# ChalmersPhotonicsLab/QAMpy

Hardware: AMD Instinct MI355X
Metric: equalised MSym/s (2-pol, 2 SPS) (higher is better)
Workload: dtype f32

## Files before the change

### qampy_amd/csrc/api.hip

```cpp
#include "common.h"
#include <stdlib.h>
#include <atomic>
#include <mutex>
#include <vector>
#include <unordered_map>
#include <string.h>

namespace qh {

thread_local hipStream_t g_stream = nullptr;
static thread_local hipStream_t g_streams[4] = {nullptr, nullptr, nullptr, nullptr};
int g_device = -1;
static thread_local std::string g_err;
static std::mutex g_mu;

void set_error(const std::string &s) { g_err = s; }

int hip_fail(hipError_t e, const char *what, const char *file, int line)
{
    g_err = std::string(hipGetErrorString(e)) + " in " + what + " (" + file + ":" + std::to_string(line) + ")";
    (void)hipGetLastError();
    return QH_ERR_HIP;
}

// ... 63 lines not shown
        QH_HIP(hipStreamCreateWithPriority(&g_streams[i], hipStreamNonBlocking, i == 2 ? prio_least : prio_greatest));
    }
    g_stream = g_streams[0];
    g_device = device;
    return QH_OK;
}

hipStream_t side_stream() { return g_stream == g_streams[0] ? g_streams[1] : g_streams[0]; }
hipStream_t helper_stream() { return g_streams[3]; }

int ensure_init()
{
    if (g_stream) return QH_OK;
    return init_device(g_device >= 0 ? g_device : 0);
}

thread_local void *g_scratch[SCRATCH_SLOTS] = {nullptr};
thread_local size_t g_scratch_n[SCRATCH_SLOTS] = {0};
thread_local unsigned g_scratch_epoch = 0;
static std::atomic<int> g_form[FORM_COUNT];
struct FormName { const char *key, *env; };
static const FormName FORM_NAMES[FORM_COUNT] = {
    {"trainer", "QAMPY_HIP_TRAINER"}, {"pit_form", "QAMPY_HIP_PIT_FORM"}, {"seg_lanes", "QAMPY_HIP_SEG_LANES"}, {"pit_probe", "QAMPY_HIP_PIT_PROBE"},
    {"bps", "QAMPY_HIP_BPS"}, {"pit_tail", "QAMPY_HIP_PIT_TAIL"}};
static int form_parse(int k, const char *v, int *out)
{
    if (!v || !v[0]) { *out = 0; return 0; }
    switch (k) {
    case FORM_TRAINER: *out = v[0] == 'd' ? 1 : (v[0] == 'l' ? 2 : (v[0] == 'i' ? 3 : (v[0] == 'a' || v[0] == '0' ? 0 : -1))); break;
    case FORM_PIT: *out = v[0] == 's' ? 1 : (v[0] == 'b' ? 2 : (v[0] == 'a' || v[0] == '0' ? 0 : -1)); break;
    case FORM_SEG_LANES: { const int n = atoi(v); *out = (n == 8 || n == 16 || n == 0) ? n : -1; break; }
    case FORM_BPS: *out = v[0] == 't' ? 1 : (v[0] == 'l' ? 2 : (v[0] == 'a' || v[0] == '0' ? 0 : -1)); break;
    case FORM_PIT_TAIL: *out = v[0] == 's' ? 1 : (v[0] == 'a' || v[0] == '0' ? 0 : -1); break;
    default: *out = atoi(v) != 0 ? 1 : 0; break;
    }
    return *out < 0 ? -1 : 0;
}
static const int g_form_env_read = [] {
    for (int k = 0; k < FORM_COUNT; k++) {
        int v = 0;
        if (form_parse(k, getenv(FORM_NAMES[k].env), &v) == 0) g_form[k].store(v);
    }
    return 0;
}();
int form(FormKey k) { return g_form[k].load(std::memory_order_relaxed); }
const char *trainer_force()
{
    switch (form(FORM_TRAINER)) {
    case 1: return "direct";
    case 2: return "lookahead";
    case 3: return "iterative";
    default: return "";
    }
}
static constexpr int POOL_CLASSES = 48, POOL_KEEP = 8;
static constexpr size_t POOL_BYTES = (size_t)24 << 30;
// ... 370 lines not shown
```

### qampy_amd/csrc/common.h

```cpp
#pragma once
#include <hip/hip_runtime.h>
#include <stdint.h>
#include <string>
#include "../../include/qampy_hip.h"

namespace qh {

extern thread_local hipStream_t g_stream;
extern int g_device;
void set_error(const std::string &s);
int hip_fail(hipError_t e, const char *what, const char *file, int line);

#define QH_HIP(call)                                                        \
    do {                                                                    \
        hipError_t _e = (call);                                             \
        if (_e != hipSuccess) return qh::hip_fail(_e, #call, __FILE__, __LINE__); \
    } while (0)

#define QH_REQUIRE(cond, msg)                                   \
    do {                                                        \
        if (!(cond)) { qh::set_error(msg); return QH_ERR_ARG; } \
    } while (0)

#define QH_WAVE_FIRST() __builtin_amdgcn_s_setprio(3)

int ensure_init();
hipStream_t side_stream();
hipStream_t helper_stream();
enum FormKey { FORM_TRAINER = 0, FORM_PIT, FORM_SEG_LANES, FORM_PIT_PROBE, FORM_BPS, FORM_PIT_TAIL, FORM_COUNT };
int form(FormKey k);
const char *trainer_force();
double gram_budget_gb();
int pit_timing_mode();
int default_tier();
double default_tier_tol();
constexpr int SCRATCH_SLOTS = 24;
constexpr int SCRATCH_TWOSTAGE = 16;
constexpr int SCRATCH_FOE = 17;
constexpr int SCRATCH_IMPAIR = 18;
constexpr int SCRATCH_PMD = 19;
constexpr int SCRATCH_TXRESP = 20;
constexpr int SCRATCH_SOS = 21;
constexpr int SCRATCH_CPR = 22;
constexpr int SCRATCH_FFT = 23;
int scratch(int slot, size_t bytes, void **p);
unsigned scratch_epoch();

int bps_twostage_recover_f32(const void *E, int nm, int64_t L, const void *angles, int A, int B, const void *symbols, int M, int N, int32_t *idx1,
                             int32_t *idx2, void *ph, void *Eout);
int bps_twostage_recover_f64(const void *E, int nm, int64_t L, const void *angles, int A, int B, const void *symbols, int M, int N, int32_t *idx1,
                             int32_t *idx2, void *ph, void *Eout);

// ... 114 lines not shown
```

### qampy_amd/csrc/train_pit.h

```cpp
#pragma once
#include <atomic>
#include <chrono>
#include <vector>
#include "train_impl.h"
#include "train_seg.h"

namespace qh {

typedef qh_pit_report PitCtrl;

constexpr double PIT_CONTRACT = 0.2;
constexpr int PIT_PROBE = 128;
constexpr int PIT_SEEDWIN = 512;
constexpr int PIT_MAXSEG = 65536;

__host__ __device__ inline int pit_symmetry(int method)
{
    switch (method) {
    case QH_M_CMA: case QH_M_SGNCMA: case QH_M_RDE: return 0;
    case QH_M_CMA2: return 2;
    default: return 4;
    }
}

// ... 27 lines not shown
    if (lane == 63) buf[wave] = x;
    __syncthreads();
    T pre = ident;
    for (int w = 0; w < wave; w++) pre = op(pre, buf[w]);
    T ex = shfl_up_any(x, 1);
    if (lane == 0) ex = ident;
    const T r = op(pre, ex);
    __syncthreads();
    return r;
}

template <typename T> __device__ __forceinline__ void block_prefix_sum(T *a, int n, T *tot)
{
    const int len = (n + 255) / 256;
    const int i0 = threadIdx.x * len, i1 = i0 + len < n ? i0 + len : n;
    T s = 0;
    for (int i = i0; i < i1; i++) s += a[i];
    T run = block_scan_excl<T>(s, [](T x, T y) { return x + y; }, (T)0, tot);
    for (int i = i0; i < i1; i++) { run += a[i]; a[i] = run; }
    __syncthreads();
}

template <typename R>
__global__ void __launch_bounds__(256) pit_setup_kernel(const Cx<R> *E, int nmodes, int64_t L, int64_t npow, int ntot, const R *mu, double gear,
                                                        double bound, double tol, PitSeg sg, PitCtrl *c, R *mu_acq)
{
    QH_WAVE_FIRST();
    __shared__ double red[256];
    double acc = 0;
    for (int k = 0; k < nmodes; k++)
        for (int64_t i = threadIdx.x; i < npow; i += 256) {
            const Cx<R> v = E[(size_t)k * L + i];
            acc += (double)v.re * v.re + (double)v.im * v.im;
        }
    red[threadIdx.x] = acc;
    __syncthreads();
    for (int s = 128; s > 0; s >>= 1) {
        if (threadIdx.x < s) red[threadIdx.x] += red[threadIdx.x + s];
        __syncthreads();
    }
    if (threadIdx.x == 0) {
        const double p = red[0] / ((double)nmodes * (double)npow);
        const double m = (double)*mu;
        double ma = gear * m;
        const double cap = bound / ((double)ntot * (p > 1e-30 ? p : 1e-30));
        if (ma > cap) ma = cap;
        if (!(ma > m)) ma = m;
        c->segments = sg.S; c->seg_len = sg.len; c->mu = m; c->mu_acq = ma; c->power = p; c->tol = tol;
        for (int q = 0; q < QH_PIT_MAXPASS; q++) { c->result_change[q] = -1; c->deviation[q] = -1; c->deviation_rms[q] = -1; c->deviation_taps[q] = -1; c->deviation_taps_worst[q] = -1; } c->passes = 0; c->converged = 0; c->acq_chunks = 0; c->acq_steps = 0; c->acq_done = 0; c->done = 0; c->diverged = 0; c->corr_on = 0; c->gain = 0; c->out_power = 0;
        for (int i = 0; i < QH_PIT_MAXPASS; i++) c->defect[i] = -1;
        for (int i = 0; i < QH_PIT_MAXCHUNK; i++) c->acq_err[i] = -1;
        *mu_acq = (R)ma;
    }
}

template <typename R>
__global__ void __launch_bounds__(256) pit_acq_monitor_kernel(const Cx<R> *err, int64_t err_pitch, int64_t step0, int64_t n, int nsel,
                                                              const int64_t *modes_dev, double plateau, PitCtrl *c, R *mu_acq, const R *mu, double floor_gear)
{
    QH_WAVE_FIRST();
    if (threadIdx.x == 0 && floor_gear >= 0) {
        const R lo = (R)((double)*mu * floor_gear), h = *mu_acq * (R)0.5;
        *mu_acq = h > lo ? h : (*mu_acq > lo ? lo : *mu_acq);
    }
    if (c->acq_done) return;
    __shared__ double red[256];
    double acc = 0;
    for (int j = 0; j < nsel; j++) {
        const Cx<R> *row = err + (size_t)modes_dev[j] * err_pitch + step0;
        for (int64_t i = threadIdx.x; i < n; i += 256) {
            const Cx<R> v = row[i];
            acc += (double)v.re * v.re + (double)v.im * v.im;
        }
    }
    red[threadIdx.x] = acc;
    __syncthreads();
    for (int s = 128; s > 0; s >>= 1) {
// ... 2 lines not shown
    }
    if (threadIdx.x == 0) {
        const double v = red[0] / ((double)n * nsel);
        const int k = c->acq_chunks;
        if (k < QH_PIT_MAXCHUNK) c->acq_err[k] = v;
        c->acq_chunks = k + 1;
        c->acq_steps = step0 + n;
        if (!(v == v) || v > 1e30) { c->diverged = 1; c->acq_done = 1; return; }
        if (k >= 1) {
            const double prev = c->acq_err[k - 1 < QH_PIT_MAXCHUNK ? k - 1 : QH_PIT_MAXCHUNK - 1];
            if (v > 100 * c->acq_err[0]) { c->diverged = 1; c->acq_done = 1; return; }
            if (v > plateau * prev) c->acq_done = 1;
        }
    }
}

template <typename R> __global__ void pit_acq_finish_kernel(Cx<R> *wx, const Cx<R> *w_start, int n, PitCtrl *c)
{
    QH_WAVE_FIRST();
    const int i = blockIdx.x * blockDim.x + threadIdx.x;
    if (c->diverged && i < n) wx[i] = w_start[i];
}

inline size_t pit_phase_pitch(int ntaps, int os, int nwin) { return (size_t)nwin + (size_t)(ntaps + os - 1) / os + 1; }
template <typename R>
__global__ void __launch_bounds__(256) pit_phase_kernel(const Cx<R> *E, int nmodes, int64_t L, int os, const Cx<R> *wx, int ntaps, PitSeg sg,
                                                        const int64_t *modes_dev, int nwin, double *z)
{
    QH_WAVE_FIRST();
    extern __shared__ __attribute__((aligned(16))) char pit_smem[];
    Cx<R> *w = reinterpret_cast<Cx<R> *>(pit_smem);
    const int ntot = nmodes * ntaps;
    const int pitch = nwin + (ntaps + os - 1) / os + 1;
    Cx<R> *xs = w + ntot;
    __shared__ double rr[256], ri[256];
    const int s = blockIdx.x, j = blockIdx.y;
    const int mode = (int)modes_dev[j];
    for (int f = threadIdx.x; f < ntot; f += 256) w[f] = wx[(size_t)mode * ntot + f];
    const int64_t st = sg.start(s);
    int64_t n = sg.steps(s);
    if (n > nwin) n = nwin;
    const int ns = n > 0 ? (int)(n - 1) * os + ntaps : 0;
    for (int k = 0; k < nmodes; k++) {
        const Cx<R> *x = E + (size_t)k * L + st * os;
        for (int g = threadIdx.x; g < ns; g += 256) xs[((size_t)k * os + g % os) * pitch + g / os] = x[g];
    }
    __syncthreads();
    double zr = 0, zi = 0;
    for (int i = threadIdx.x; i < n; i += 256) {
        R yr = 0, yi = 0;
        for (int k = 0; k < nmodes; k++) {
            const Cx<R> *wk = w + k * ntaps;
            for (int r = 0; r < os; r++) {
                const Cx<R> *xp = xs + ((size_t)k * os + r) * pitch + i;
                int u = 0;
                for (int t = r; t < ntaps; t += os, u++) {
                    const Cx<R> a = xp[u], b = wk[t];
                    yr = fma_(a.re, b.re, fma_(-a.im, b.im, yr));
                    yi = fma_(a.re, b.im, fma_(a.im, b.re, yi));
                }
            }
        }
        const double y2r = (double)yr * yr - (double)yi * yi, y2i = 2.0 * yr * yi;
        zr += y2r * y2r - y2i * y2i;
        zi += 2.0 * y2r * y2i;
    }
    rr[threadIdx.x] = zr; ri[threadIdx.x] = zi;
    __syncthreads();
    for (int q = 128; q > 0; q >>= 1) {
        if (threadIdx.x < q) { rr[threadIdx.x] += rr[threadIdx.x + q]; ri[threadIdx.x] += ri[threadIdx.x + q]; }
        __syncthreads();
    }
    if (threadIdx.x == 0) { z[2 * ((size_t)s * gridDim.y + j)] = rr[0]; z[2 * ((size_t)s * gridDim.y + j) + 1] = ri[0]; }
}

static __global__ void __launch_bounds__(256) pit_unwrap_kernel(const double *z, int S, int nsel, double *rot, double *phi, int *jump)
{
    QH_WAVE_FIRST();
    __shared__ int ptot[512];
    const double q = 1.5707963267948966;
    phi += (size_t)blockIdx.x * S; jump += (size_t)blockIdx.x * S;
    for (int j = blockIdx.x; j <= (int)blockIdx.x; j++) {
        for (int s = threadIdx.x; s < S; s += 256) {
            const double zr = z[2 * ((size_t)s * nsel + j)], zi = z[2 * ((size_t)s * nsel + j) + 1];
            phi[s] = (zr == 0 && zi == 0) ? 0.0 : (double)atan2f((float)-zi, (float)-zr) / 4;
        }
        __syncthreads();
        for (int s = threadIdx.x; s < S; s += 256) jump[s] = s == 0 ? 0 : (int)rint((phi[s - 1] - phi[s]) / q);
        __syncthreads();
        block_prefix_sum<int>(jump, S, ptot);
        for (int s = threadIdx.x; s < S; s += 256) {
            const double p = phi[s] + q * (jump[s] & 3);
            float sn, cs;
            sincosf((float)p, &sn, &cs);
            rot[2 * ((size_t)s * nsel + j)] = cs;
            rot[2 * ((size_t)s * nsel + j) + 1] = -sn;
        }
        __syncthreads();
    }
}

template <typename R>
__global__ void __launch_bounds__(256) pit_seed_kernel(const Cx<R> *wx, int nmodes, int ntot, const int64_t *modes_dev, int nsel, const double *rot, Cx<R> *X,
                                                       const Cx<R> *w0, Cx<R> *Y, PitCtrl *c)
{
    QH_WAVE_FIRST();
    const int s = blockIdx.x;
    const int n = nmodes * ntot;
    if (s == 0 && c) {
        if (threadIdx.x == 0) { c->done = 0; c->converged = 0; c->passes = 0; }
        for (int q = threadIdx.x; q < QH_PIT_MAXPASS; q += 256) {
            c->result_change[q] = -1; c->deviation[q] = -1; c->deviation_rms[q] = -1; c->deviation_taps[q] = -1; c->deviation_taps_worst[q] = -1; c->defect[q] = -1;
        }
    }
    const bool exact0 = s == 0 && w0 != nullptr;
    for (int e = threadIdx.x; e < n; e += 256) {
        const int row = e / ntot;
        Cx<R> v = exact0 ? w0[e] : wx[e];
        if (rot && !exact0) {
            for (int j = 0; j < nsel; j++)
                if ((int)modes_dev[j] == row) {
                    const double c = rot[2 * ((size_t)s * nsel + j)], d = rot[2 * ((size_t)s * nsel + j) + 1];
                    const double vr = (double)v.re * c - (double)v.im * d, vi = (double)v.re * d + (double)v.im * c;
                    v = Cx<R>{(R)vr, (R)vi};
                    break;
                }
        }
        X[(size_t)s * n + e] = v;
        Y[(size_t)s * n + e] = v;
    }
}

template <typename R>
__global__ void __launch_bounds__(PIT_PROBE) pit_defect_kernel(const Cx<R> *E, int nmodes, int64_t L, int os, int ntaps, PitSeg sg, int64_t TrSyms,
                                                                const int64_t *modes_dev, const Cx<R> *X, const Cx<R> *Y, int sym, const PitCtrl *c, double *dfc, double *pw, double *gph,
                                                                const Cx<R> *wx_prev)
{
    QH_WAVE_FIRST();
    if (c->done) return;
    extern __shared__ __attribute__((aligned(16))) char pit_smem[];
    Cx<R> *wa = reinterpret_cast<Cx<R> *>(pit_smem);
    const int ntot = nmodes * ntaps;
    Cx<R> *wb = wa + ntot;
    const int pitch = PIT_PROBE + (ntaps + os - 1) / os + 1;
    Cx<R> *xs = wb + ntot;
    __shared__ double red[4][PIT_PROBE];
    const int b = blockIdx.x + 1, j = blockIdx.y;
    const int mode = (int)modes_dev[j];
    const size_t wset = (size_t)nmodes * ntot;
    const bool result_probe = b == sg.S;
    for (int f = threadIdx.x; f < ntot; f += PIT_PROBE) {
        wa[f] = result_probe ? wx_prev[(size_t)mode * ntot + f] : X[(size_t)b * wset + (size_t)mode * ntot + f];
        wb[f] = Y[(size_t)(b - 1) * wset + (size_t)mode * ntot + f];
// ... 1723 lines not shown

struct PitPrepLayout { size_t ctrl, mu_acq, modes, wx, w0, err, gram, total; int64_t err_pitch; };
template <typename R> inline PitPrepLayout pit_prep_layout(int nmodes, int ntaps, int64_t acq_steps)
{
    PitPrepLayout l;
    auto up = [](size_t x) { return (x + 255) / 256 * 256; };
    const size_t wset = (size_t)nmodes * nmodes * ntaps * sizeof(Cx<R>);
    l.err_pitch = (acq_steps + LA_B + 63) / 64 * 64;
    l.ctrl = 0; l.mu_acq = up(sizeof(PitCtrl)); l.modes = l.mu_acq + 64; l.wx = up(l.modes + 128); l.w0 = up(l.wx + wset);
    l.err = up(l.w0 + wset); l.gram = up(l.err + (size_t)nmodes * l.err_pitch * sizeof(Cx<R>));
    l.total = up(l.gram + gram_bytes<R>(l.err_pitch));
    return l;
}
template <typename R> __global__ void __launch_bounds__(256) pit_adopt_kernel(Cx<R> *wx, const Cx<R> *wx_prep, int n, const PitCtrl *p, PitCtrl *c, R *mu_acq, const R *mu_acq_prep)
{
    QH_WAVE_FIRST();
    const int i = blockIdx.x * blockDim.x + threadIdx.x;
    if (!p->diverged && i < n) wx[i] = wx_prep[i];
    if (i == 0) {
        c->acq_chunks = p->acq_chunks; c->acq_steps = p->acq_steps; c->acq_done = 1; c->diverged = p->diverged; c->mu_acq = p->mu_acq;
        for (int q = 0; q < QH_PIT_MAXCHUNK; q++) c->acq_err[q] = p->acq_err[q];
        *mu_acq = *mu_acq_prep;
    }
}
template <typename R>
int pit_prepare(const void *E, int nmodes, int64_t L, int64_t TrSyms, int os, const R *mu_dev, const void *wx0, int ntaps, const int64_t *modes, int nsel,
                const void *symbols, int64_t nsy, int method, const qh_pit_opts *opts, void *prep, size_t prep_bytes)
{
    int rc = ensure_init();
    if (rc) return rc;
    if ((rc = train_args_ok("pit prepare", method, nmodes, ntaps, os, TrSyms, 1, nsel, nsy, modes))) return rc;
    QH_REQUIRE(opts && prep, "pit prepare: options and a preparation buffer are needed");
    QH_REQUIRE(TrSyms >= 1, "pit prepare: bad sizes");
    QH_REQUIRE((TrSyms - 1) * os + ntaps <= L, "pit prepare: field shorter than TrSyms*os + ntaps");
    const qh_pit_opts &o = *opts;
    QH_REQUIRE(o.acquire != 0 && o.adaptive == 0 && o.segments > 1 && o.mu_hint > 0 && o.acq_chunk > 0 && o.head_steps == 0 && !o.exchange,
               "pit prepare: not preparable (a cold fixed-step sweep with segments, mu_hint and acq_chunk given)");
    const int ntot = nmodes * ntaps;
    const PitPlan pl = pit_plan(o, TrSyms, 0, o.segments, false, o.acq_chunk);
    const PitSeg &sg = pl.sg;
    QH_REQUIRE(sg.S >= 2, "pit prepare: not preparable (nothing to parallelise)");
    const char *not_prep = "pit prepare: not preparable (throughput-form passes, block-form acquisition, blind error function)";
    QH_REQUIRE(!(method == QH_M_SBD || method == QH_M_MDDMA || method == QH_M_DD || method == QH_M_SBD_DATA), not_prep);
    TrainerForm f;
    if ((rc = trainer_form<R>(f, FORM_PASSES, method, 0, nmodes, ntaps, os, sg.len, (int64_t)sg.S * nsel, symbols, nsy, modes, nsel))) return rc;
    QH_REQUIRE(f.seg && f.block && la_shape_ok(nmodes, ntaps, os), not_prep);
// ... 87 lines not shown
        QH_REQUIRE(!o.exchange, "train_equaliser: a capture split over processes takes no exact head");
        head = (int64_t)o.head_steps / LA_B * LA_B;
        if (head > TrSyms) head = TrSyms / LA_B * LA_B;
        o.acquire = 0;
    }
    int64_t seg_want = 2048;
    if (adaptive && !(method == QH_M_SBD || method == QH_M_MDDMA || method == QH_M_DD)) {
        const int64_t t = ((TrSyms - head) / 512 + LA_B - 1) / LA_B * LA_B;
        if (t > seg_want) seg_want = t;
    }
    if (S == 0 && adaptive) S = (int)((TrSyms - head) / seg_want < PIT_MAXSEG ? (TrSyms - head) / seg_want : PIT_MAXSEG);
    if (S == 0) {
        R mu_h = (R)o.mu_hint;
        if (!(o.mu_hint > 0)) {
            QH_HIP(hipMemcpyAsync(&mu_h, mu_dev, sizeof(R), hipMemcpyDeviceToHost, g_stream));
            QH_HIP(hipStreamSynchronize(g_stream));
        }
        S = pit_auto_segments(TrSyms, (double)mu_h, nsel, o.acquire);
    }
    PitPlan pl = pit_plan(o, TrSyms, head, S, adaptive, o.acquire ? o.acq_chunk : 0);
    const PitSeg &sg = pl.sg;
    if (zero_err) QH_HIP(hipMemsetAsync(err, 0, (size_t)nmodes * TrSyms * Niter * sizeof(Cx<R>), g_stream));
    const int64_t npow = L < 4096 ? L : 4096;
    hipLaunchKernelGGL((pit_setup_kernel<R>), dim3(1), dim3(256), 0, g_stream, (const Cx<R> *)E, nmodes, L, npow, ntot, (const R *)mu_dev, pl.gear, pl.bound, tol, sg, ctrl, mu_acq);
    QH_HIP(hipGetLastError());
    if (TrSyms == 0 || Niter == 0) return QH_OK;
    if (sg.S < 2) {
        const double zero = 0;
        QH_HIP(hipMemcpyAsync(&ctrl->defect[0], &zero, sizeof(double), hipMemcpyHostToDevice, g_stream));
        return exact_form(ctrl, adaptive ? 1 : 0, 0, gram, 1);
    }

    TrainerForm f;
    if ((rc = trainer_form<R>(f, FORM_PASSES, method, adaptive, nmodes, ntaps, os, sg.len, (int64_t)sg.S * nsel, symbols, nsy, modes, nsel))) return rc;
    if (adaptive && !f.seg) return exact_form(ctrl, 1, 0, nullptr, 0);
    const bool decision = method == QH_M_SBD || method == QH_M_MDDMA || method == QH_M_DD;
    const bool seg_form = f.seg, use_bi = f.use_bi, block_form = f.block, pair_tab = f.pair_tab;
    const bool split = o.exchange != nullptr;
    const int own_first = split ? o.seg_first : 0, own_count = split ? o.seg_count : sg.S;
    const bool xchg_async = split && o.exchange_on_stream != 0;
    if (split) {
        QH_REQUIRE(seg_form, "train_equaliser: a capture split over processes needs the throughput form of the passes (>= 512 chains, supported tap layout)");
        QH_REQUIRE(own_first >= 0 && own_count >= 0 && own_first + own_count <= sg.S, "train_equaliser: owned segments outside the segment grid");
        QH_REQUIRE(Niter == 1, "train_equaliser: a capture split over processes is trained in one sweep");
    }

    const size_t wset = (size_t)nmodes * ntot;
// ... 10 lines not shown
    float *devmax = (float *)(uw_jump + (size_t)sg.S * nsel);
    const int ndev = (int)((nsj + 63) / 64);
    unsigned *ticket = (unsigned *)(devmax + 4 * (size_t)ndev);
    PitInit init{};
    init.z[0] = ticket; init.zn[0] = sizeof(unsigned);
    R *ad_rS = nullptr, *ad_rE = nullptr;
    Cx<R> *ad_eS = nullptr, *ad_eE = nullptr, *ad_errh = nullptr;
    float *ad_M = nullptr, *ad_chg = nullptr, *ad_rP = nullptr, *ad_dP = nullptr;
    if (!adaptive && head > 0) {
        void *ab = nullptr;
        if ((rc = scratch(13, (size_t)nmodes * head * sizeof(Cx<R>) + 64, &ab))) return rc;
        ad_errh = (Cx<R> *)ab;
    }
    if (adaptive) {
        void *ab = nullptr;
        const size_t nS = ((size_t)sg.S + 15) / 16 * 16;
        if ((rc = scratch(13, nS * (2 * sizeof(R) + 2 * sizeof(Cx<R>) + 3 * sizeof(float)) + 64 + (size_t)nmodes * head * sizeof(Cx<R>), &ab))) return rc;
        ad_eS = (Cx<R> *)ab; ad_eE = ad_eS + nS; ad_errh = ad_eE + nS;
        ad_rS = (R *)(ad_errh + (size_t)nmodes * head); ad_rE = ad_rS + nS;
        ad_M = (float *)(ad_rE + nS); ad_rP = ad_M + nS; ad_dP = ad_rP + nS; ad_chg = ad_dP + nS;
    }
    init.modes_dev = modes_dev; init.nsel = nsel;
    for (int j = 0; j < 16; j++) init.modes[j] = j < nsel ? modes[j] : 0;
    const bool prepared = o.prepared != nullptr && o.acquire && !adaptive && head == 0 && Niter >= 1;
    const bool need_mu = adaptive || !(o.mu_hint > 0), need_acq = o.acquire && !(o.acq_chunk > 0) && !prepared;
    R mu_acq_h = 0;
    if (need_acq) QH_HIP(hipMemcpyAsync(&mu_acq_h, mu_acq, sizeof(R), hipMemcpyDeviceToHost, g_stream));
    R mu_host = need_mu ? (R)1 : (R)o.mu_hint;
    if (need_mu) QH_HIP(hipMemcpyAsync(&mu_host, mu_dev, sizeof(R), hipMemcpyDeviceToHost, g_stream));
    if (need_mu || need_acq) QH_HIP(hipStreamSynchronize(g_stream));
    if (!adaptive && !(mu_host != 0))
        return exact_form(ctrl, 0, 0, gram, 0);
    if (o.acquire && !(o.acq_chunk > 0)) pl.acquisition(o, TrSyms, pit_acq_chunk(mu_acq_h));

    const int64_t amax = pl.amax;
    void *G = const_cast<void *>(gram);
    if (prepared) QH_REQUIRE(seg_form && o.acq_chunk > 0, "train_equaliser: a prepared acquisition belongs to throughput-form passes with acq_chunk given (qh_pit_prepare_*_dev said so)");
    if (block_form && !G && (!seg_form || amax > 0) && !prepared) {
        const int64_t n = seg_form ? pl.ngram : TrSyms;
        rc = pair_tab ? gram_build<R>(E, nmodes, L, os, ntaps, n, &G) : gram_cur_build<R>(E, nmodes, L, os, ntaps, n, &G);
        if (rc) return rc;
    }
    const int64_t g_per_step = pair_tab ? LA_B : GRAM_TRI / 2 / LA_B;

    const int ncol = sg.S * nsel;
    const double *lam = nullptr;
    const Zf *Vb = nullptr;
    Zf *Dz[2] = {nullptr, nullptr};
// ... 40 lines not shown
        QH_HIP(hipFuncSetAttribute((const void *)pit_cgemm_kernel<R, true>, hipFuncAttributeMaxDynamicSharedMemorySize, 160 * 1024 - 256));
        QH_HIP(hipFuncSetAttribute((const void *)pit_cgemm_kernel<R, false>, hipFuncAttributeMaxDynamicSharedMemorySize, 160 * 1024 - 256));
        QH_HIP(hipFuncSetAttribute((const void *)pit_basis_mfma_kernel<R, 0>, hipFuncAttributeMaxDynamicSharedMemorySize, 128 * 1024));
        QH_HIP(hipFuncSetAttribute((const void *)pit_basis_mfma_kernel<R, 1>, hipFuncAttributeMaxDynamicSharedMemorySize, 128 * 1024));
        QH_HIP(hipFuncSetAttribute((const void *)pit_tail_kernel<R>, hipFuncAttributeMaxDynamicSharedMemorySize, 128 * 1024));
        gemm_attr.store(true, std::memory_order_release);
    }

    LaArgs<R> la = la_args<R>(E, L, nmodes, ntaps, os, modes, nsel, method, symbols, nsy, mu_dev, err, TrSyms * Niter);
    la.G = (const GramPair<R> *)G; la.gpair = pair_tab ? 1 : 0; la.wx_cs = (int64_t)wset;
    la.dd_general = f.dd_general;
    f.alphabet(la);
    const TrainArgs<R> ta = train_args<R>(E, L, nmodes, ntaps, os, TrSyms, Niter, modes, nsel, method, symbols, nsy, mu_dev, err);

    PitTiming &tm = pit_timing();
    tm.npass = 0; tm.acq_ms = 0;
    bool acq_timed = false;
    PitEvents &ev = pit_events();
    QH_REQUIRE(ev.ok, "train_equaliser: no pinned memory for the pass flags");
    const bool redo_ok = o.exact_redo_off == 0;
    bool fell_back = false;
    if (redo_ok && !adaptive) { init.cd[0] = w_call; init.cs[0] = wx; init.cn[0] = (unsigned)wbytes; }
    if (o.acquire && Niter > 0) { init.cd[1] = w_start; init.cs[1] = wx; init.cn[1] = (unsigned)wbytes; }
    hipLaunchKernelGGL(pit_init_kernel, dim3(32), dim3(256), 0, g_stream, init);
    QH_HIP(hipGetLastError());
    for (int it = 0; it < Niter; it++) {
        if (it == 0 && prepared) {
            const PitPrepLayout lay = pit_prep_layout<R>(nmodes, ntaps, amax);
            const char *pb = (const char *)o.prepared;
            hipLaunchKernelGGL((pit_adopt_kernel<R>), dim3((unsigned)((wset + 255) / 256)), dim3(256), 0, g_stream, (Cx<R> *)wx, (const Cx<R> *)(pb + lay.wx), (int)wset,
                               (const PitCtrl *)(pb + lay.ctrl), ctrl, mu_acq, (const R *)(pb + lay.mu_acq));
            QH_HIP(hipGetLastError());
        } else if (it == 0 && o.acquire) {
            if (pl.nchunks > 0) { QH_HIP(hipEventRecord(ev.t0[PIT_NEV - 1], g_stream)); acq_timed = true; }
            if ((rc = pit_acq_enqueue<R>(pl, block_form ? &la : nullptr, use_bi, &ta, (Cx<R> *)wx, (Cx<R> *)err, TrSyms * Niter, ctrl, mu_acq, mu_dev,
                                         modes_dev, nsel))) return rc;
            if (pl.nchunks > 0) QH_HIP(hipEventRecord(ev.t1[PIT_NEV - 1], g_stream));
            hipLaunchKernelGGL((pit_acq_finish_kernel<R>), dim3((unsigned)((wset + 255) / 256)), dim3(256), 0, g_stream, (Cx<R> *)wx, (const Cx<R> *)w_start, (int)wset, ctrl);
            QH_HIP(hipGetLastError());
        }
        if (adaptive) {
            QH_HIP(hipMemcpyAsync(w_start, wx, wbytes, hipMemcpyDeviceToDevice, g_stream));
            QH_HIP(hipMemcpyAsync(ad_chg + 1, mu_dev, sizeof(R), hipMemcpyDeviceToDevice, g_stream));
            if ((rc = train_dev<R>(E, nmodes, L, head, 1, os, mu_dev, wx, ntaps, modes, 1, 1, symbols, nsy, method, ad_errh, 0, nullptr))) return rc;
            QH_HIP(hipMemcpyAsync((Cx<R> *)err + (size_t)modes[0] * TrSyms, ad_errh + (size_t)modes[0] * head, (size_t)head * sizeof(Cx<R>), hipMemcpyDeviceToDevice, g_stream));
            hipLaunchKernelGGL((pit_adapt_init_kernel<R>), dim3((sg.S + 255) / 256), dim3(256), 0, g_stream, (const R *)mu_dev, (const Cx<R> *)(ad_errh + (size_t)modes[0] * head + head - 1),
                               sg.S, ad_rS, ad_eS);
            QH_HIP(hipGetLastError());
        }
        if (!adaptive && head > 0) {
            if ((rc = train_dev<R>(E, nmodes, L, head, 1, os, mu_dev, wx, ntaps, modes, nsel, 0, symbols, nsy, method, ad_errh, 0, nullptr))) return rc;
            for (int j = 0; j < nsel; j++)
                QH_HIP(hipMemcpyAsync((Cx<R> *)err + (size_t)modes[j] * TrSyms * Niter + (size_t)it * TrSyms, ad_errh + (size_t)modes[j] * head, (size_t)head * sizeof(Cx<R>),
                                      hipMemcpyDeviceToDevice, g_stream));
        }
        const double *rot_use = nullptr;
        if (seed_phase) {
            int nwin = PIT_SEEDWIN;
            auto phase_lds = [&](int nw) { return ((size_t)ntot + (size_t)nmodes * os * pit_phase_pitch(ntaps, os, nw)) * sizeof(Cx<R>); };
            while (nwin > 32 && phase_lds(nwin) > 60 * 1024) nwin /= 2;
            QH_REQUIRE(phase_lds(nwin) <= 60 * 1024, "train_equaliser: phase seeding does not fit the LDS for this filter shape (pass phase_seed = 0)");
            hipLaunchKernelGGL((pit_phase_kernel<R>), dim3(sg.S, nsel), dim3(256), phase_lds(nwin), g_stream, (const Cx<R> *)E, nmodes, L, os,
                               (const Cx<R> *)wx, ntaps, sg, (const int64_t *)modes_dev, nwin, z);
            hipLaunchKernelGGL(pit_unwrap_kernel, dim3(nsel), dim3(256), 0, g_stream, (const double *)z, sg.S, nsel, rot, uw_phi, uw_jump);
            rot_use = rot;
        }
        const Cx<R> *w_exact = o.start == 1 ? nullptr : ((it == 0 && o.acquire) ? (const Cx<R> *)w_start : (const Cx<R> *)wx);
        hipLaunchKernelGGL((pit_seed_kernel<R>), dim3(sg.S), dim3(256), 0, g_stream, (const Cx<R> *)wx, nmodes, ntot, (const int64_t *)modes_dev, nsel, rot_use, X, w_exact, Y, ctrl);
        if (ssb) {
            ma.sg = sg; ma.rot = rot_use;
            static thread_local hipEvent_t ev_seed = nullptr, ev_model = nullptr;
            if (!ev_seed) { QH_HIP(hipEventCreateWithFlags(&ev_seed, hipEventDisableTiming)); QH_HIP(hipEventCreateWithFlags(&ev_model, hipEventDisableTiming)); }
            hipStream_t ss = helper_stream();
            QH_HIP(hipEventRecord(ev_seed, g_stream));
            QH_HIP(hipStreamWaitEvent(ss, ev_seed, 0));
            hipLaunchKernelGGL((pit_model_kernel<R, 0>), dim3(PIT_MODB), dim3(256), 0, ss, ma);
            hipLaunchKernelGGL((pit_model_kernel<R, 1>), dim3(PIT_MODB), dim3(256), 0, ss, ma);
            QH_HIP(hipEventRecord(ev_model, ss));
            model_event = ev_model;
        }
        QH_HIP(hipGetLastError());
        const int timing_mode = pit_timing_mode();
        auto decide_args = [&](int p, const float *dm, const float2 *ye, float2 *yprev, int ne, int ncol_e, int corr_wanted) {
            PitDecideArgs<R> d;
            d.dfc = dfc; d.pw = pw; d.nb = (int)((sg.S - 1) * nsel); d.Ylast = (const Cx<R> *)(Y + (size_t)(sg.S - 1) * wset); d.n = (int)wset; d.wx = (Cx<R> *)wx; d.c = ctrl;
            d.host_view = &ev.hview[2 * p]; d.nrow = nsel; d.devmax = dm; d.ndev = ndev; d.safety = safety; d.Ye = ye; d.Yprev = yprev; d.ne = ne; d.ncol_e = ncol_e;
            d.theta = theta; d.modes_dev = (const int64_t *)modes_dev; d.ntot_w = ntot; d.S = (int)sg.S; d.sym = sym; d.corr_wanted = corr_wanted;
            d.extra = adaptive ? (const float *)ad_chg : nullptr;
            d.Dfin = (ye && !adaptive) ? (const float2 *)Dz[1] : nullptr; d.Vfin = (const float2 *)Vb; d.lam_fin = lam;
            d.stall_from = o.correction == 0 ? QH_PIT_MAXPASS : (adaptive ? 5 : 2);
            return d;
        };
        auto timed = [&](int p) { return timing_mode == 2 || (timing_mode == 1 && p == 1); };
        int back_done_for = 0;
        auto enqueue_pass = [&](int p) -> int {
            ((volatile float *)ev.hview)[2 * p] = -1.f;
            PitFuse<R> fz;
            fz.X = X; fz.Y = Y; fz.theta = theta; fz.modes_dev = (const int64_t *)modes_dev; fz.nmodes = nmodes; fz.nsel = nsel;
            fz.damp = (adaptive && p > 1) ? ad_damp : 1.f;
            fz.x_only = tail_fused ? 1 : 0;
            if (p > 0 && tail_fused && back_done_for == p) {
// ... 24 lines not shown
                for (int j = 0; j < 16; j++) sa.modes[j] = j < nsel ? modes[j] : 0;
                sa.skip = &ctrl->done;
                sa.q_first = own_first * nsel; sa.q_count = split ? own_count * nsel : 0;
                pit_last_launch().form = 1;
                if (!split || own_count > 0) { int r = launch_seg<R>(sa, method, adaptive); if (r) return r; }
                if (adaptive) hipLaunchKernelGGL((pit_adapt_scan_kernel<R>), dim3(1), dim3(1024), 0, g_stream, ad_rS, (const R *)ad_rE, ad_eS, (const Cx<R> *)ad_eE, sg.S, ad_chg, (const PitCtrl *)ctrl, ad_relax, ad_rP, ad_dP, ad_newton);
            } else if (block_form) {
                LaArgs<R> ls = la;
                ls.TrSyms = sg.len; ls.nch = sg.S; ls.wx = Y; ls.err_off = (int64_t)it * TrSyms; ls.seg = 1; ls.seg_extra = sg.extra; ls.seg_tail = sg.tail;
                ls.skip = &ctrl->done;
                pit_last_launch() = PitLaunch{use_bi ? 2 : 3, 0, 0, 0, 0, 0};
                if (sg.begin > 0) {
                    ls.E = (const Cx<R> *)E + sg.begin * os; ls.L = L - sg.begin * os; ls.err_off += sg.begin;
                    ls.G = (const GramPair<R> *)G + sg.begin * g_per_step;
                }
                { int r = use_bi ? launch_bi<R>(ls) : launch_la<R>(ls); if (r) return r; }
            } else {
                TrainArgs<R> ts = ta;
                ts.wx = Y; ts.nseg = sg.S; ts.seg_begin = sg.begin; ts.seg_len = sg.len; ts.seg_extra = sg.extra; ts.seg_tail = sg.tail; ts.seg_iter = it; ts.skip = &ctrl->done;
                pit_last_launch() = PitLaunch{4, 0, 0, 0, 0, 0};
                { int r = launch_any<R>(ts); if (r) return r; }
            }
            if (timed(p)) QH_HIP(hipEventRecord(ev.t1[p], g_stream));
            if (split) {
                if (own_first > 0) QH_HIP(hipMemsetAsync(Y, 0, (size_t)own_first * wbytes, g_stream));
                if (own_first + own_count < sg.S)
                    QH_HIP(hipMemsetAsync(Y + (size_t)(own_first + own_count) * wset, 0, (size_t)(sg.S - own_first - own_count) * wbytes, g_stream));
                if (!xchg_async) QH_HIP(hipStreamSynchronize(g_stream));
                if (o.exchange(o.exchange_user, Y, (size_t)sg.S * wbytes) != 0) { set_error("train_equaliser: the exchange callback failed"); return QH_ERR_ARG; }
            }
            const int nbnd = (int)((sg.S - 1) * nsel);
            if (eig) {
                if (o.basis && pit_basis_sync().pending) {
                    QH_HIP(hipStreamWaitEvent(g_stream, pit_basis_sync().out, 0));
                    pit_basis_sync().pending = false;
                }
                auto forward2 = [&](const Cx<R> *src, Zf *dst, const Cx<R> *src2, Zf *dst2) {
                    PitFuse<R> f2 = fz;
                    f2.T2 = src2; f2.Out2 = reinterpret_cast<float2 *>(dst2);
                    hipLaunchKernelGGL((pit_basis_mfma_kernel<R, 0>), dim3(2 * ((ncol + PIT_MC - 1) / PIT_MC)), dim3(pit_mfma_threads(ntot)), pit_mfma_lds(ntot), g_stream, Vb, src, (const Zf *)nullptr, dst, ntot, ncol, (const PitCtrl *)ctrl, f2);
                };
                if (p == 0 && model_event) QH_HIP(hipStreamWaitEvent(g_stream, model_event, 0));
                forward2((const Cx<R> *)X, Xe, (const Cx<R> *)Y, Ye);
                hipLaunchKernelGGL(pit_bound_kernel, dim3((nbnd + nsel + 3) / 4), dim3(256), 0, g_stream, (const Zf *)Xe, (const Zf *)Ye, (const Zf *)Yprev, lam, ntot, sg.S, nsel, sym,
                                   (const PitCtrl *)ctrl, dfc, pw, gph, ualpha);
                hipLaunchKernelGGL((pit_gauge_kernel<R>), dim3(ssb ? 2 : 1), dim3(PIT_GT_THREADS), 0, g_stream, (const double *)gph, sg.S, nsel, ctrl, theta, (const double *)pw,
// ... 194 lines not shown
```

Before: 1237.

## Merge PIT prologue kernels and add windowed phase-seed kernel

```diff
diff --git a/qampy_amd/csrc/api.hip b/qampy_amd/csrc/api.hip
--- a/qampy_amd/csrc/api.hip
+++ b/qampy_amd/csrc/api.hip
@@ -109,7 +109,7 @@
 struct FormName { const char *key, *env; };
 static const FormName FORM_NAMES[FORM_COUNT] = {
     {"trainer", "QAMPY_HIP_TRAINER"}, {"pit_form", "QAMPY_HIP_PIT_FORM"}, {"seg_lanes", "QAMPY_HIP_SEG_LANES"}, {"pit_probe", "QAMPY_HIP_PIT_PROBE"},
-    {"bps", "QAMPY_HIP_BPS"}, {"pit_tail", "QAMPY_HIP_PIT_TAIL"}};
+    {"bps", "QAMPY_HIP_BPS"}, {"pit_tail", "QAMPY_HIP_PIT_TAIL"}, {"pit_prologue", "QAMPY_HIP_PIT_PROLOGUE"}};
 static int form_parse(int k, const char *v, int *out)
 {
     if (!v || !v[0]) { *out = 0; return 0; }
@@ -118,7 +118,7 @@
     case FORM_PIT: *out = v[0] == 's' ? 1 : (v[0] == 'b' ? 2 : (v[0] == 'a' || v[0] == '0' ? 0 : -1)); break;
     case FORM_SEG_LANES: { const int n = atoi(v); *out = (n == 8 || n == 16 || n == 0) ? n : -1; break; }
     case FORM_BPS: *out = v[0] == 't' ? 1 : (v[0] == 'l' ? 2 : (v[0] == 'a' || v[0] == '0' ? 0 : -1)); break;
-    case FORM_PIT_TAIL: *out = v[0] == 's' ? 1 : (v[0] == 'a' || v[0] == '0' ? 0 : -1); break;
+    case FORM_PIT_TAIL: case FORM_PIT_PROLOGUE: *out = v[0] == 's' ? 1 : (v[0] == 'a' || v[0] == '0' ? 0 : -1); break;
     default: *out = atoi(v) != 0 ? 1 : 0; break;
     }
     return *out < 0 ? -1 : 0;
diff --git a/qampy_amd/csrc/common.h b/qampy_amd/csrc/common.h
--- a/qampy_amd/csrc/common.h
+++ b/qampy_amd/csrc/common.h
@@ -27,7 +27,7 @@
 int ensure_init();
 hipStream_t side_stream();
 hipStream_t helper_stream();
-enum FormKey { FORM_TRAINER = 0, FORM_PIT, FORM_SEG_LANES, FORM_PIT_PROBE, FORM_BPS, FORM_PIT_TAIL, FORM_COUNT };
+enum FormKey { FORM_TRAINER = 0, FORM_PIT, FORM_SEG_LANES, FORM_PIT_PROBE, FORM_BPS, FORM_PIT_TAIL, FORM_PIT_PROLOGUE, FORM_COUNT };
 int form(FormKey k);
 const char *trainer_force();
 double gram_budget_gb();
diff --git a/qampy_amd/csrc/train_pit.h b/qampy_amd/csrc/train_pit.h
--- a/qampy_amd/csrc/train_pit.h
+++ b/qampy_amd/csrc/train_pit.h
@@ -73,10 +73,9 @@
 }
 
 template <typename R>
-__global__ void __launch_bounds__(256) pit_setup_kernel(const Cx<R> *E, int nmodes, int64_t L, int64_t npow, int ntot, const R *mu, double gear,
-                                                        double bound, double tol, PitSeg sg, PitCtrl *c, R *mu_acq)
-{
-    QH_WAVE_FIRST();
+__device__ __forceinline__ void pit_setup_body(const Cx<R> *E, int nmodes, int64_t L, int64_t npow, int ntot, const R *mu, double gear,
+                                               double bound, double tol, PitSeg sg, PitCtrl *c, R *mu_acq)
+{
     __shared__ double red[256];
     double acc = 0;
     for (int k = 0; k < nmodes; k++)
@@ -104,6 +103,13 @@
         *mu_acq = (R)ma;
     }
 }
+template <typename R>
+__global__ void __launch_bounds__(256) pit_setup_kernel(const Cx<R> *E, int nmodes, int64_t L, int64_t npow, int ntot, const R *mu, double gear,
+                                                        double bound, double tol, PitSeg sg, PitCtrl *c, R *mu_acq)
+{
+    QH_WAVE_FIRST();
+    pit_setup_body<R>(E, nmodes, L, npow, ntot, mu, gear, bound, tol, sg, c, mu_acq);
+}
 
 template <typename R>
 __global__ void __launch_bounds__(256) pit_acq_monitor_kernel(const Cx<R> *err, int64_t err_pitch, int64_t step0, int64_t n, int nsel,
@@ -152,10 +158,12 @@
     if (c->diverged && i < n) wx[i] = w_start[i];
 }
 
+__device__ __forceinline__ double pit_seed_phi(double zr, double zi) { return (zr == 0 && zi == 0) ? 0.0 : (double)atan2f((float)-zi, (float)-zr) / 4; }
+
 inline size_t pit_phase_pitch(int ntaps, int os, int nwin) { return (size_t)nwin + (size_t)(ntaps + os - 1) / os + 1; }
 template <typename R>
 __global__ void __launch_bounds__(256) pit_phase_kernel(const Cx<R> *E, int nmodes, int64_t L, int os, const Cx<R> *wx, int ntaps, PitSeg sg,
-                                                        const int64_t *modes_dev, int nwin, double *z)
+                                                        const int64_t *modes_dev, int nwin, double *z, double *phi = nullptr)
 {
     QH_WAVE_FIRST();
     extern __shared__ __attribute__((aligned(16))) char pit_smem[];
@@ -201,7 +209,116 @@
         if (threadIdx.x < q) { rr[threadIdx.x] += rr[threadIdx.x + q]; ri[threadIdx.x] += ri[threadIdx.x + q]; }
         __syncthreads();
     }
-    if (threadIdx.x == 0) { z[2 * ((size_t)s * gridDim.y + j)] = rr[0]; z[2 * ((size_t)s * gridDim.y + j) + 1] = ri[0]; }
+    if (threadIdx.x == 0) {
+        z[2 * ((size_t)s * gridDim.y + j)] = rr[0]; z[2 * ((size_t)s * gridDim.y + j) + 1] = ri[0];
+        if (phi) phi[(size_t)s * gridDim.y + j] = pit_seed_phi(rr[0], ri[0]);
+    }
+}
+
+constexpr int PIT_PW_OUT = 2, PIT_PW_TAPS = 8;
+inline int pit_phase_win_pitch(int ntaps, int os, int nwin)
+{
+    const int nu = (ntaps + os - 1) / os;
+    return (nwin + (nu + PIT_PW_TAPS - 1) / PIT_PW_TAPS * PIT_PW_TAPS + 2) & ~1;
+}
+inline size_t pit_phase_win_lds(int nmodes, int ntaps, int os, int nwin) { return ((size_t)nmodes * os * pit_phase_win_pitch(ntaps, os, nwin) + nwin) * sizeof(Cx<float>); }
+static __global__ void __launch_bounds__(256) pit_phase_win_kernel(const Cx<float> *__restrict__ E, int nmodes, int64_t L, int os, const Cx<float> *__restrict__ wx, int ntaps,
+                                                                   PitSeg sg, const int64_t *__restrict__ modes_dev, int nwin, int pitch, double *__restrict__ z, double *__restrict__ phi)
+{
+    QH_WAVE_FIRST();
+    typedef float v2 __attribute__((ext_vector_type(2)));
+    typedef float v4 __attribute__((ext_vector_type(4)));
+    extern __shared__ __attribute__((aligned(16))) char pit_smem[];
+    Cx<float> *xs = reinterpret_cast<Cx<float> *>(pit_smem);
+    Cx<float> *yo = xs + (size_t)nmodes * os * pitch;
+    __shared__ double rr[256], ri[256];
+    const int s = blockIdx.x, j = blockIdx.y;
+    const Cx<float> *wm = wx + (size_t)modes_dev[j] * ((size_t)nmodes * ntaps);
+    const int64_t st = sg.start(s);
+    int64_t n64 = sg.steps(s);
+    if (n64 > nwin) n64 = nwin;
+    const int n = (int)n64;
+    const int ns = n > 0 ? (n - 1) * os + ntaps : 0;
+    const bool os_pow2 = (os & (os - 1)) == 0;
+    const int os_sh = __ffs(os) - 1;
+    for (int k = 0; k < nmodes; k++) {
+        const Cx<float> *x = E + (size_t)k * L + st * os;
+        Cx<float> *xk = xs + (size_t)k * os * pitch;
+        for (int g0 = threadIdx.x; g0 < ns; g0 += 4 * 256) {
+            Cx<float> v[4];
+#pragma unroll
+            for (int q = 0; q < 4; q++)
+                if (g0 + q * 256 < ns) v[q] = ldg(x + g0 + q * 256);
+#pragma unroll
+            for (int q = 0; q < 4; q++) {
+                const int g = g0 + q * 256;
+                if (g < ns) {
+                    const int u = os_pow2 ? g >> os_sh : g / os, r = g - u * os;
+                    stg(xk + (size_t)r * pitch + u, v[q]);
+                }
+            }
+        }
+    }
+    __syncthreads();
+    auto cmac = [](v2 &acc, const Cx<float> a, const Cx<float> b) {
+        acc = __builtin_elementwise_fma(v2{-a.im, a.im}, v2{b.im, b.re}, acc);
+        acc = __builtin_elementwise_fma(v2{a.re, a.re}, v2{b.re, b.im}, acc);
+    };
+    for (int i = PIT_PW_OUT * threadIdx.x; i < n; i += PIT_PW_OUT * 256) {
+        v2 y0{0.f, 0.f}, y1{0.f, 0.f};
+        for (int k = 0; k < nmodes; k++) {
+            const Cx<float> *wk = wm + k * ntaps;
+            for (int r = 0; r < os; r++) {
+                const Cx<float> *xp = xs + ((size_t)k * os + r) * pitch + i;
+                const int nt = (ntaps - r + os - 1) / os;
+                for (int u0 = 0; u0 < nt; u0 += PIT_PW_TAPS) {
+                    Cx<float> x[PIT_PW_TAPS + 2];
+#pragma unroll
+                    for (int q = 0; q < PIT_PW_TAPS / 2 + 1; q++) {
+                        const v4 p = *reinterpret_cast<const v4 *>(xp + u0 + 2 * q);
+                        x[2 * q] = Cx<float>{p.x, p.y}; x[2 * q + 1] = Cx<float>{p.z, p.w};
+                    }
+                    const Cx<float> *wt = wk + r + (size_t)u0 * os;
+                    if (u0 + PIT_PW_TAPS <= nt) {
+#pragma unroll
+                        for (int uu = 0; uu < PIT_PW_TAPS; uu++) {
+                            const Cx<float> b = wt[uu * os];
+                            cmac(y0, x[uu], b);
+                            cmac(y1, x[uu + 1], b);
+                        }
+                    } else {
+#pragma unroll
+                        for (int uu = 0; uu < PIT_PW_TAPS; uu++)
+                            if (u0 + uu < nt) {
+                                const Cx<float> b = wt[uu * os];
+                                cmac(y0, x[uu], b);
+                                cmac(y1, x[uu + 1], b);
+                            }
+                    }
+                }
+            }
+        }
+        yo[i] = Cx<float>{y0.x, y0.y};
+        if (i + 1 < n) yo[i + 1] = Cx<float>{y1.x, y1.y};
+    }
+    __syncthreads();
+    double zr = 0, zi = 0;
+    for (int i = threadIdx.x; i < n; i += 256) {
+        const float yr = yo[i].re, yi = yo[i].im;
+        const double y2r = (double)yr * yr - (double)yi * yi, y2i = 2.0 * yr * yi;
+        zr += y2r * y2r - y2i * y2i;
+        zi += 2.0 * y2r * y2i;
+    }
+    rr[threadIdx.x] = zr; ri[threadIdx.x] = zi;
+    __syncthreads();
+    for (int q = 128; q > 0; q >>= 1) {
+        if (threadIdx.x < q) { rr[threadIdx.x] += rr[threadIdx.x + q]; ri[threadIdx.x] += ri[threadIdx.x + q]; }
+        __syncthreads();
+    }
+    if (threadIdx.x == 0) {
+        z[2 * ((size_t)s * gridDim.y + j)] = rr[0]; z[2 * ((size_t)s * gridDim.y + j) + 1] = ri[0];
+        if (phi) phi[(size_t)s * gridDim.y + j] = pit_seed_phi(rr[0], ri[0]);
+    }
 }
 
 static __global__ void __launch_bounds__(256) pit_unwrap_kernel(const double *z, int S, int nsel, double *rot, double *phi, int *jump)
@@ -230,11 +347,10 @@
     }
 }
 
-template <typename R>
-__global__ void __launch_bounds__(256) pit_seed_kernel(const Cx<R> *wx, int nmodes, int ntot, const int64_t *modes_dev, int nsel, const double *rot, Cx<R> *X,
-                                                       const Cx<R> *w0, Cx<R> *Y, PitCtrl *c)
-{
-    QH_WAVE_FIRST();
+template <typename R, typename RotAt>
+__device__ __forceinline__ void pit_seed_body(const Cx<R> *wx, int nmodes, int ntot, const int64_t *modes_dev, int nsel, bool rot, RotAt rot_at, Cx<R> *X,
+                                              const Cx<R> *w0, Cx<R> *Y, PitCtrl *c)
+{
     const int s = blockIdx.x;
     const int n = nmodes * ntot;
     if (s == 0 && c) {
@@ -250,7 +366,8 @@
         if (rot && !exact0) {
             for (int j = 0; j < nsel; j++)
                 if ((int)modes_dev[j] == row) {
-                    const double c = rot[2 * ((size_t)s * nsel + j)], d = rot[2 * ((size_t)s * nsel + j) + 1];
+                    double c, d;
+                    rot_at(j, c, d);
                     const double vr = (double)v.re * c - (double)v.im * d, vi = (double)v.re * d + (double)v.im * c;
                     v = Cx<R>{(R)vr, (R)vi};
                     break;
@@ -259,6 +376,49 @@
         X[(size_t)s * n + e] = v;
         Y[(size_t)s * n + e] = v;
     }
+}
+template <typename R>
+__global__ void __launch_bounds__(256) pit_seed_kernel(const Cx<R> *wx, int nmodes, int ntot, const int64_t *modes_dev, int nsel, const double *rot, Cx<R> *X,
+                                                       const Cx<R> *w0, Cx<R> *Y, PitCtrl *c)
+{
+    QH_WAVE_FIRST();
+    const int s = blockIdx.x;
+    pit_seed_body<R>(wx, nmodes, ntot, modes_dev, nsel, rot != nullptr,
+                     [&](int j, double &cr, double &ci) { cr = rot[2 * ((size_t)s * nsel + j)]; ci = rot[2 * ((size_t)s * nsel + j) + 1]; }, X, w0, Y, c);
+}
+constexpr int PIT_FOLD_MAX = 8192, PIT_SEEDU_THREADS = 1024;
+template <typename R>
+__global__ void __launch_bounds__(PIT_SEEDU_THREADS) pit_seed_unwrap_kernel(const Cx<R> *wx, int nmodes, int ntot, const int64_t *modes_dev, int nsel, const double *__restrict__ phi,
+                                                                            double *rot, Cx<R> *X, const Cx<R> *w0, Cx<R> *Y, PitCtrl *c)
+{
+    QH_WAVE_FIRST();
+    __shared__ int jump[16];
+    __shared__ double rc[16], rd[16];
+    const int s = blockIdx.x;
+    const double q = 1.5707963267948966;
+    if (threadIdx.x < 16) jump[threadIdx.x] = 0;
+    __syncthreads();
+    const int ne = (s + 1) * nsel;
+#pragma unroll 4
+    for (int e = nsel + threadIdx.x; e < ne; e += PIT_SEEDU_THREADS) {
+        const double d = phi[e - nsel] - phi[e];
+        if (fabs(d) < 0.7) continue;
+        const int jm = (int)rint(d / q);
+        if (jm) atomicAdd(&jump[e % nsel], jm);
+    }
+    __syncthreads();
+    if ((int)threadIdx.x < nsel) {
+        const int j = threadIdx.x;
+        const double p = phi[(size_t)s * nsel + j] + q * (jump[j] & 3);
+        float sn, cs;
+        sincosf((float)p, &sn, &cs);
+        rc[j] = cs; rd[j] = -sn;
+        rot[2 * ((size_t)s * nsel + j)] = cs;
+        rot[2 * ((size_t)s * nsel + j) + 1] = -sn;
+    }
+    __syncthreads();
+    if (threadIdx.x < 256)
+        pit_seed_body<R>(wx, nmodes, ntot, modes_dev, nsel, true, [&](int j, double &cr, double &ci) { cr = rc[j]; ci = rd[j]; }, X, w0, Y, c);
 }
 
 template <typename R>
@@ -2028,6 +2188,43 @@
         for (int q = 0; q < QH_PIT_MAXCHUNK; q++) c->acq_err[q] = p->acq_err[q];
         *mu_acq = *mu_acq_prep;
     }
+}
+template <typename R> struct PitOpen {
+    const Cx<R> *E; int nmodes; int64_t L, npow; int ntot; const R *mu; double gear, bound, tol; PitSeg sg; PitCtrl *c; R *mu_acq;
+    PitInit init;
+    uint64_t *wx; const uint64_t *wx_prep; unsigned adopt_n; const PitCtrl *prep; const R *mu_acq_prep;
+};
+template <typename R> __global__ void __launch_bounds__(256) pit_open_kernel(PitOpen<R> a)
+{
+    QH_WAVE_FIRST();
+    if (blockIdx.x == 0) {
+        pit_setup_body<R>(a.E, a.nmodes, a.L, a.npow, a.ntot, a.mu, a.gear, a.bound, a.tol, a.sg, a.c, a.mu_acq);
+        if (threadIdx.x == 0 && a.wx_prep) {
+            const PitCtrl *p = a.prep;
+            PitCtrl *c = a.c;
+            c->acq_chunks = p->acq_chunks; c->acq_steps = p->acq_steps; c->acq_done = 1; c->diverged = p->diverged; c->mu_acq = p->mu_acq;
+            for (int q = 0; q < QH_PIT_MAXCHUNK; q++) c->acq_err[q] = p->acq_err[q];
+            *a.mu_acq = *a.mu_acq_prep;
+        }
+        return;
+    }
+    const PitInit &in = a.init;
+    const unsigned t = (blockIdx.x - 1) * 256 + threadIdx.x, nt = (gridDim.x - 1) * 256;
+#pragma unroll
+    for (int r = 0; r < 3; r++)
+        if (in.z[r]) for (unsigned i = t; i < in.zn[r] / 4; i += nt) reinterpret_cast<uint32_t *>(in.z[r])[i] = 0u;
+    const bool adopt = a.wx_prep && !a.prep->diverged;
+    unsigned nmax = adopt ? a.adopt_n : 0u;
+#pragma unroll
+    for (int r = 0; r < 2; r++)
+        if (in.cd[r] && in.cn[r] / 8 > nmax) nmax = in.cn[r] / 8;
+    for (unsigned i = t; i < nmax; i += nt) {
+#pragma unroll
+        for (int r = 0; r < 2; r++)
+            if (in.cd[r] && i < in.cn[r] / 8) reinterpret_cast<uint64_t *>(in.cd[r])[i] = reinterpret_cast<const uint64_t *>(in.cs[r])[i];
+        if (adopt && i < a.adopt_n) a.wx[i] = a.wx_prep[i];
+    }
+    if ((int)t < in.nsel) in.modes_dev[t] = in.modes[t];
 }
 template <typename R>
 int pit_prepare(const void *E, int nmodes, int64_t L, int64_t TrSyms, int os, const R *mu_dev, const void *wx0, int ntaps, const int64_t *modes, int nsel,
@@ -2161,7 +2358,12 @@
     const PitSeg &sg = pl.sg;
     if (zero_err) QH_HIP(hipMemsetAsync(err, 0, (size_t)nmodes * TrSyms * Niter * sizeof(Cx<R>), g_stream));
     const int64_t npow = L < 4096 ? L : 4096;
-    hipLaunchKernelGGL((pit_setup_kernel<R>), dim3(1), dim3(256), 0, g_stream, (const Cx<R> *)E, nmodes, L, npow, ntot, (const R *)mu_dev, pl.gear, pl.bound, tol, sg, ctrl, mu_acq);
+    const bool prepared = o.prepared != nullptr && o.acquire && !adaptive && head == 0 && Niter >= 1;
+    const bool need_mu = adaptive || !(o.mu_hint > 0), need_acq = o.acquire && !(o.acq_chunk > 0) && !prepared;
+    const bool new_prologue = form(FORM_PIT_PROLOGUE) == 0;
+    const bool open_merged = new_prologue && !need_mu && (R)o.mu_hint != 0 && !need_acq && TrSyms > 0 && Niter > 0 && sg.S >= 2;
+    if (!open_merged)
+        hipLaunchKernelGGL((pit_setup_kernel<R>), dim3(1), dim3(256), 0, g_stream, (const Cx<R> *)E, nmodes, L, npow, ntot, (const R *)mu_dev, pl.gear, pl.bound, tol, sg, ctrl, mu_acq);
     QH_HIP(hipGetLastError());
     if (TrSyms == 0 || Niter == 0) return QH_OK;
     if (sg.S < 2) {
@@ -2218,8 +2420,6 @@
     }
     init.modes_dev = modes_dev; init.nsel = nsel;
     for (int j = 0; j < 16; j++) init.modes[j] = j < nsel ? modes[j] : 0;
-    const bool prepared = o.prepared != nullptr && o.acquire && !adaptive && head == 0 && Niter >= 1;
-    const bool need_mu = adaptive || !(o.mu_hint > 0), need_acq = o.acquire && !(o.acq_chunk > 0) && !prepared;
     R mu_acq_h = 0;
     if (need_acq) QH_HIP(hipMemcpyAsync(&mu_acq_h, mu_acq, sizeof(R), hipMemcpyDeviceToHost, g_stream));
     R mu_host = need_mu ? (R)1 : (R)o.mu_hint;
@@ -2306,10 +2506,23 @@
     bool fell_back = false;
     if (redo_ok && !adaptive) { init.cd[0] = w_call; init.cs[0] = wx; init.cn[0] = (unsigned)wbytes; }
     if (o.acquire && Niter > 0) { init.cd[1] = w_start; init.cs[1] = wx; init.cn[1] = (unsigned)wbytes; }
-    hipLaunchKernelGGL(pit_init_kernel, dim3(32), dim3(256), 0, g_stream, init);
+    if (open_merged) {
+        PitOpen<R> op{};
+        op.E = (const Cx<R> *)E; op.nmodes = nmodes; op.L = L; op.npow = npow; op.ntot = ntot; op.mu = (const R *)mu_dev; op.gear = pl.gear; op.bound = pl.bound; op.tol = tol;
+        op.sg = sg; op.c = ctrl; op.mu_acq = mu_acq; op.init = init;
+        if (prepared) {
+            const PitPrepLayout lay = pit_prep_layout<R>(nmodes, ntaps, pl.amax);
+            const char *pb = (const char *)o.prepared;
+            op.wx = (uint64_t *)wx; op.wx_prep = (const uint64_t *)(pb + lay.wx); op.adopt_n = (unsigned)(wbytes / 8);
+            op.prep = (const PitCtrl *)(pb + lay.ctrl); op.mu_acq_prep = (const R *)(pb + lay.mu_acq);
+        }
+        hipLaunchKernelGGL((pit_open_kernel<R>), dim3(33), dim3(256), 0, g_stream, op);
+    } else
+        hipLaunchKernelGGL(pit_init_kernel, dim3(32), dim3(256), 0, g_stream, init);
     QH_HIP(hipGetLastError());
     for (int it = 0; it < Niter; it++) {
-        if (it == 0 && prepared) {
+        if (it == 0 && prepared && open_merged) {
+        } else if (it == 0 && prepared) {
             const PitPrepLayout lay = pit_prep_layout<R>(nmodes, ntaps, amax);
             const char *pb = (const char *)o.prepared;
             hipLaunchKernelGGL((pit_adopt_kernel<R>), dim3((unsigned)((wset + 255) / 256)), dim3(256), 0, g_stream, (Cx<R> *)wx, (const Cx<R> *)(pb + lay.wx), (int)wset,
@@ -2339,28 +2552,47 @@
                                       hipMemcpyDeviceToDevice, g_stream));
         }
         const double *rot_use = nullptr;
+        bool seed_unwrap = false;
         if (seed_phase) {
             int nwin = PIT_SEEDWIN;
             auto phase_lds = [&](int nw) { return ((size_t)ntot + (size_t)nmodes * os * pit_phase_pitch(ntaps, os, nw)) * sizeof(Cx<R>); };
             while (nwin > 32 && phase_lds(nwin) > 60 * 1024) nwin /= 2;
             QH_REQUIRE(phase_lds(nwin) <= 60 * 1024, "train_equaliser: phase seeding does not fit the LDS for this filter shape (pass phase_seed = 0)");
-            hipLaunchKernelGGL((pit_phase_kernel<R>), dim3(sg.S, nsel), dim3(256), phase_lds(nwin), g_stream, (const Cx<R> *)E, nmodes, L, os,
-                               (const Cx<R> *)wx, ntaps, sg, (const int64_t *)modes_dev, nwin, z);
-            hipLaunchKernelGGL(pit_unwrap_kernel, dim3(nsel), dim3(256), 0, g_stream, (const double *)z, sg.S, nsel, rot, uw_phi, uw_jump);
+            seed_unwrap = new_prologue && nsj <= (size_t)PIT_FOLD_MAX;
+            double *phi_out = seed_unwrap ? uw_phi : nullptr;
+            bool win = false;
+            if constexpr (sizeof(R) == 4)
+                if (new_prologue && nwin == PIT_SEEDWIN && pit_phase_win_lds(nmodes, ntaps, os, nwin) <= 60 * 1024) {
+                    win = true;
+                    hipLaunchKernelGGL(pit_phase_win_kernel, dim3(sg.S, nsel), dim3(256), pit_phase_win_lds(nmodes, ntaps, os, nwin), g_stream, (const Cx<float> *)E, nmodes, L, os,
+                                       (const Cx<float> *)wx, ntaps, sg, (const int64_t *)modes_dev, nwin, pit_phase_win_pitch(ntaps, os, nwin), z, phi_out);
+                }
+            if (!win)
+                hipLaunchKernelGGL((pit_phase_kernel<R>), dim3(sg.S, nsel), dim3(256), phase_lds(nwin), g_stream, (const Cx<R> *)E, nmodes, L, os,
+                                   (const Cx<R> *)wx, ntaps, sg, (const int64_t *)modes_dev, nwin, z, phi_out);
+            if (!seed_unwrap) hipLaunchKernelGGL(pit_unwrap_kernel, dim3(nsel), dim3(256), 0, g_stream, (const double *)z, sg.S, nsel, rot, uw_phi, uw_jump);
             rot_use = rot;
         }
         const Cx<R> *w_exact = o.start == 1 ? nullptr : ((it == 0 && o.acquire) ? (const Cx<R> *)w_start : (const Cx<R> *)wx);
-        hipLaunchKernelGGL((pit_seed_kernel<R>), dim3(sg.S), dim3(256), 0, g_stream, (const Cx<R> *)wx, nmodes, ntot, (const int64_t *)modes_dev, nsel, rot_use, X, w_exact, Y, ctrl);
-        if (ssb) {
-            ma.sg = sg; ma.rot = rot_use;
-            static thread_local hipEvent_t ev_seed = nullptr, ev_model = nullptr;
-            if (!ev_seed) { QH_HIP(hipEventCreateWithFlags(&ev_seed, hipEventDisableTiming)); QH_HIP(hipEventCreateWithFlags(&ev_model, hipEventDisableTiming)); }
+        if (seed_unwrap)
+            hipLaunchKernelGGL((pit_seed_unwrap_kernel<R>), dim3(sg.S), dim3(PIT_SEEDU_THREADS), 0, g_stream, (const Cx<R> *)wx, nmodes, ntot, (const int64_t *)modes_dev, nsel, (const double *)uw_phi, rot,
+                               X, w_exact, Y, ctrl);
+        else
+            hipLaunchKernelGGL((pit_seed_kernel<R>), dim3(sg.S), dim3(256), 0, g_stream, (const Cx<R> *)wx, nmodes, ntot, (const int64_t *)modes_dev, nsel, rot_use, X, w_exact, Y, ctrl);
+        static thread_local hipEvent_t ev_seed = nullptr, ev_model = nullptr;
+        auto enqueue_model = [&]() -> int {
             hipStream_t ss = helper_stream();
-            QH_HIP(hipEventRecord(ev_seed, g_stream));
             QH_HIP(hipStreamWaitEvent(ss, ev_seed, 0));
             hipLaunchKernelGGL((pit_model_kernel<R, 0>), dim3(PIT_MODB), dim3(256), 0, ss, ma);
             hipLaunchKernelGGL((pit_model_kernel<R, 1>), dim3(PIT_MODB), dim3(256), 0, ss, ma);
             QH_HIP(hipEventRecord(ev_model, ss));
+            return QH_OK;
+        };
+        if (ssb) {
+            ma.sg = sg; ma.rot = rot_use;
+            if (!ev_seed) { QH_HIP(hipEventCreateWithFlags(&ev_seed, hipEventDisableTiming)); QH_HIP(hipEventCreateWithFlags(&ev_model, hipEventDisableTiming)); }
+            QH_HIP(hipEventRecord(ev_seed, g_stream));
+            if (!new_prologue && (rc = enqueue_model())) return rc;
             model_event = ev_model;
         }
         QH_HIP(hipGetLastError());
@@ -2431,6 +2663,7 @@
                 { int r = launch_any<R>(ts); if (r) return r; }
             }
             if (timed(p)) QH_HIP(hipEventRecord(ev.t1[p], g_stream));
+            if (p == 0 && ssb && new_prologue) { int r = enqueue_model(); if (r) return r; }
             if (split) {
                 if (own_first > 0) QH_HIP(hipMemsetAsync(Y, 0, (size_t)own_first * wbytes, g_stream));
                 if (own_first + own_count < sg.S)
```

After: 1248, median of 6. About the same (+1.0%).
